# lingya/titan

Hardware: AMD Instinct MI355X
Metric: BFS GTEPS + PageRank s/iter, RMAT scale-24 (1 GPU) and scale-27 (1/2/4/8 GPU) (higher is better)
Workload: dtype int32 (BFS levels); f64 (PageRank)

## Files before the change

### titan_amd/csrc/api_msbfs.cpp

```cpp
#include <algorithm>
#include <cstdio>
#include <cstring>
#include "ctx.hpp"

using namespace tgo;

namespace tgo {

int ms_alloc(tgo_ctx* ctx) {
    Scratch& s = ctx->sc;
    if (s.ms_vis) return TGO_OK;
    const int64_t n = ctx->g.n;
    HIP_TRY(dev_alloc(ctx, s.ms_vis, n + 1));
    HIP_TRY(dev_alloc(ctx, s.ms_fr, n + 1));
    HIP_TRY(dev_alloc(ctx, s.ms_nx, n + 1));
    HIP_TRY(dev_alloc(ctx, s.ms_lvl, n * kLevelPlanes + 1));
    HIP_TRY(dev_alloc(ctx, s.ms_fbm, (n + 63) / 64 + 1));
    HIP_TRY(dev_alloc(ctx, s.ms_seeds, TGO_MAX_SOURCES));
    HIP_TRY(dev_alloc(ctx, s.ms_stat, 2 * TGO_MAX_SOURCES));
    HIP_TRY(dev_alloc(ctx, s.ms_srcent, TGO_MAX_SOURCES));
    ctx->st.device_bytes = ctx->dev_bytes;
    return TGO_OK;
}

double ms_split_of(const tgo_ctx* ctx) {
    static const double env = env_double("TGO_MS_SPLIT", 0.005);
    return tuned(ctx->tune.f64(TGO_TUNE_MS_SPLIT), env);
}
double ms_stay_of(const tgo_ctx* ctx) {
    static const double env = env_clamped("TGO_MS_STAY", kMsStayDefault, 0.0, HUGE_VAL);
    return tuned(ctx->tune.f64(TGO_TUNE_MS_STAY), env);
// ... 63 lines not shown
    s.ms_masks_zero = false;
    if (!masks_zero) HIP_TRY(hipMemsetAsync(s.ms_fr, 0, n * 8, st));
    s.ms_nplanes = 0;
    HIP_TRY(k_ms_seed(s.ms_seeds, nseeds, s.ms_vis, s.ms_fr, INT64_MAX, st));
    HIP_TRY(k_degree_i64(push, s.q[0], static_cast<int64_t>(uniq.size()), s.qdeg, st));
    const uint64_t full = nseeds == 64 ? ~0ULL : ((1ULL << nseeds) - 1ULL);
    const int64_t total = pull.nlists > 1 ? g.out.nnz + g.in.nnz : (scope == TGO_SCOPE_IN_E ? g.out.nnz : g.in.nnz);
    static const double ms_alpha = env_double("TGO_MS_ALPHA", 12.0);
    static const bool trace = trace_on();
    static const int32_t filter_from = env_double("TGO_MS_FILTER", 0.0) != 0.0
        ? 0 : static_cast<int32_t>(env_double("TGO_MS_FILTER_FROM", -1.0));
    const bool filter = filter_from >= 0 && filter_from < n;
    const double split_frac = tgo::ms_split_of(ctx);
    const double stay_gamma = tgo::ms_stay_of(ctx), sparse_frac = tgo::ms_sparse_of(ctx);
    const int64_t head = tgo::ms_head_of(ctx);
    int64_t qlen = static_cast<int64_t>(uniq.size());
    int64_t mf = 0;
    int64_t reached = qlen;
    bool srcent_ready = false;
    static const double push_light = env_double("TGO_MS_PUSH_LIGHT", 1.0 / 16.0);
    static const bool push_probe = env_double("TGO_MS_PUSH_PROBE", 1.0) != 0.0;
    static const int push_range_log2 = static_cast<int>(env_double("TGO_MS_PUSH_RANGE", 0.0));
    static const int64_t push_range_min = static_cast<int64_t>(env_double("TGO_MS_PUSH_RANGE_MIN", 1048576.0));
    const int depth = std::min(max_depth, 65534);
    uint64_t* fr = s.ms_fr;
    uint64_t* nx = s.ms_nx;
    int cur = 0, levels = 0;
    bool queued = true;
    bool pulled = false;
    bool cnt_zero = false;
    bool nx_clean = masks_zero;
    int64_t prev_mf = 0;
    int64_t mu = -1;
    bool level0_sparse = false, last_sparse = false;
    unsigned long long se_pub[TGO_MAX_SOURCES] = {};
    const volatile unsigned long long* hw = host_words(ctx);
    for (int L = 0; L < depth && qlen > 0; ++L) {
        const bool stay = pulled && mu >= 0 && stay_gamma > 0.0 &&
                          static_cast<double>(mu) <= stay_gamma * static_cast<double>(mf);
        const bool use_pull = stay || static_cast<double>(mf) * ms_alpha > static_cast<double>(total);
        DevSpan span(st, "msbfs.level", {"level", L}, {"pull", use_pull ? 1 : 0});
        if ((rc = ms_planes_for(ctx, L + 1))) return rc;
        const bool queued_before = queued;
        if (!use_pull && !queued) {
            if (!cnt_zero) HIP_TRY(hipMemsetAsync(s.cnt, 0, sizeof(Counters), st));
            HIP_TRY(k_ms_queue(push, g.n_active, fr, s.q[cur], s.qdeg, s.cnt, st));
        }
        queued = !use_pull;
        const bool prev_pull = pulled;
        pulled = use_pull;
        bool sums = false;
        if (!use_pull && !queued_before) cnt_zero = false;
        bool sparse_level = false;
        bool count_open = false;
        if (use_pull) {
            if (!cnt_zero) HIP_TRY(hipMemsetAsync(s.cnt, 0, sizeof(Counters), st));
            cnt_zero = true;
// ... 49 lines not shown
            }
            if (filter) HIP_TRY(k_ms_fbitmap(fr, n, s.ms_fbm, st));
            MsColdSplit cs;
            static const bool cold_env = env_double("TGO_MS_COLD", 0.0) != 0.0;
            const int64_t cold = ctx->tune.i64(TGO_TUNE_MS_COLD);
            const bool cold_on = tuned_on(cold, cold_env);
            if (cold_on && !prev_pull && !filter) {
                if ((rc = ms_cold_layout(ctx, scope, pull, cold))) return rc;
                if (g.msc_C > 0) {
                    cs.hot_lim = g.msc_hot;
                    cs.acc = s.ms_cacc;
                    cs.need = s.ms_need;
                }
            }
            count_open = stay_gamma > 0.0 && !cs.acc && mf < prev_mf;
            HIP_TRY(k_ms_pull(pull, push, g.n_active, full, fr, filter ? s.ms_fbm : nullptr, s.ms_vis, nx,
                              ms_planes(ctx), s.cnt, L + 1, st, filter ? filter_from : 0, full & ~sparse,
                              sparse ? nx : nullptr, cs, count_open, cs.acc ? 0 : head));
            if (cs.acc) {
                HIP_TRY(k_ms_cold(g.msc_adj, g.msc_row, g.msc_C, fr, s.ms_need, s.ms_cacc, st));
                HIP_TRY(k_ms_finish(push, g.n_active, full, s.ms_vis, nx, sparse ? nx : nullptr, ms_planes(ctx), s.cnt,
                                    L + 1, s.ms_need, s.ms_cacc, st));
            }
        } else {
            HIP_TRY(k_level_prep(cnt_zero ? nullptr : s.cnt, nx, nx_clean ? 0 : g.n_active, s.qdeg + qlen, st));
            cnt_zero = true;
            const int64_t rng = static_cast<int64_t>(1) << std::min(40, std::max(0, push_range_log2));
            const int64_t nr = (g.n_active + rng - 1) / rng;
            const bool ranged = push_range_log2 > 0 && mf >= push_range_min && nr > 1 &&
                                (nr + 1) * qlen <= kMsRangePairs && nr * qlen + 1 <= n + 2;
            sparse_level = sparse_frac > 0.0 && !ranged &&
                           (L == 0 || static_cast<double>(mf) <= sparse_frac * static_cast<double>(g.n_active));
            sums = split_frac > 0.0 && (L == 0 || static_cast<double>(mf) * ms_alpha * 64.0 > static_cast<double>(total));
// ... 22 lines not shown
            } else if (next_pull) {
                HIP_TRY(k_ms_settle_count(push, g.n_active, s.ms_vis, nx, ms_planes(ctx), s.cnt, L + 1, st,
                                          sums ? s.ms_srcent : nullptr));
                queued = false;
            } else {
                HIP_TRY(k_ms_settle(push, g.n_active, s.ms_vis, nx, ms_planes(ctx), s.q[cur ^ 1], s.qdeg, s.cnt, L + 1,
                                    st, sums ? s.ms_srcent : nullptr));
            }
        }
        srcent_ready = !use_pull && sums;
        {
            unsigned long long seq = 0;
            if ((rc = turn_begin(ctx, seq, sums ? s.ms_srcent : nullptr))) return rc;
            cnt_zero = true;
            if (sums) s.ms_srcent_zero = true;
            if (L + 1 < depth && (rc = ms_planes_for(ctx, L + 2))) return rc;
            if ((rc = wait_publish(ctx, seq))) return rc;
        }
        qlen = static_cast<int64_t>(s.hcnt->qlen);
        prev_mf = mf;
        mf = static_cast<int64_t>(s.hcnt->mf);
        mu = count_open ? static_cast<int64_t>(s.hcnt->open) : -1;
        if (sums)
            for (int r = 0; r < TGO_MAX_SOURCES; ++r) se_pub[r] = hw[kPublishExtra + r];
        reached += qlen;
        nx_clean = sparse_level;
        last_sparse = sparse_level;
        if (L == 0) level0_sparse = sparse_level;
        if (trace) std::fprintf(stderr, "[tgo] ms level %d %s -> %lld vertices, %lld entries, %llu source-bits%s\n", L,
                                use_pull ? "pull" : "push", (long long)qlen, (long long)mf, s.hcnt->red[0],
                                use_pull ? (stay ? " (stayed in pull)" : "") : (sparse_level ? " (sparse)" : ""));
        if (trace && count_open) std::fprintf(stderr, "[tgo]   %lld list entries of still-open vertices\n", (long long)mu);
        static const bool diag = env_double("TGO_MS_DIAG", 0.0) != 0.0;
        if (trace && diag && use_pull) {
            unsigned long long d[kMsDiagWords] = {};
            HIP_TRY(k_ms_diag_take(d, st));
            std::fprintf(stderr, "[tgo]   pull: %llu entries examined, %llu hot / %llu cold mask gathers, %llu open vertices, "
                         "%llu stopped early; long lists: %llu, %llu entries examined (%llu hot / %llu cold gathers), "
                         "%llu stopped early\n", d[0], d[1], d[2], d[3], d[4], d[6], d[5], d[8], d[9], d[7]);
            std::fprintf(stderr, "[tgo]   long lists covered within 4 / 8 / 16 / 32 / 64 entries: %llu / %llu / %llu / %llu / %llu, "
                         "later %llu, never %llu (head %lld)\n", d[10], d[11], d[12], d[13], d[14], d[15], d[16],
                         static_cast<long long>(head));
        }
        std::swap(fr, nx);
        cur ^= 1;
        ++levels;
    }
    if (qlen > 0 && max_depth > depth)
// ... 73 lines not shown
```

### titan_amd/csrc/ctx.hpp

```cpp
#pragma once
#include <algorithm>
#include <atomic>
#include <memory>
#include <string>
#include <utility>
#include <vector>
#include <hip/hip_runtime_api.h>
#include "engine.hpp"
#include "trace.hpp"
#include "tuning.hpp"
#include "../../include/titan_gpu_olap_part.h"

struct tgo_ctx {
    tgo_options opts{};
    hipStream_t stream = nullptr;
    bool own_stream = false;
    std::string err;
    tgo::RowStaging staging;
    tgo::DevGraph g;
    bool loaded = false;
    std::vector<int64_t> titan_id;
    std::vector<int32_t> perm;
    bool id_sorted = false;
    std::vector<std::pair<int64_t, int32_t>> id_index;
// ... 244 lines not shown
int run_bfs(tgo_ctx* ctx, int64_t seed, int max_depth, int scope);

int titan_ids_by_index(tgo_ctx* ctx);

int tri_forward_lists(tgo_ctx* ctx);

int ms_alloc(tgo_ctx* ctx);
double ms_split_of(const tgo_ctx* ctx);
double ms_stay_of(const tgo_ctx* ctx);
double ms_sparse_of(const tgo_ctx* ctx);
int64_t ms_head_of(const tgo_ctx* ctx);
int run_ms_sweep(tgo_ctx* ctx, const int64_t* seeds, int32_t nseeds, int32_t max_depth, int32_t scope, int32_t flags);

inline LevelPlanes ms_planes(tgo_ctx* ctx) { return LevelPlanes{ctx->sc.ms_lvl, ctx->g.n}; }

inline int ms_planes_for(tgo_ctx* ctx, int32_t level) {
    Scratch& s = ctx->sc;
    while (s.ms_nplanes < kLevelPlanes && (level >> s.ms_nplanes) != 0) {
        HIP_TRY(hipMemsetAsync(s.ms_lvl + static_cast<int64_t>(s.ms_nplanes) * ctx->g.n, 0,
                               ctx->g.n * sizeof(uint64_t), ctx->stream));
        ++s.ms_nplanes;
    }
    return TGO_OK;
}

}

#include "program.hpp"
```

### titan_amd/csrc/engine.hpp

```cpp
#pragma once
#include <algorithm>
#include <cstdint>
#include <string>
#include <vector>
#include <hip/hip_runtime_api.h>
#include "../../include/titan_gpu_olap.h"
#include "env.hpp"

namespace tgo {

template <class T>
struct DevArray {
    T* p = nullptr;
    int64_t n = -1;
    DevArray() = default;
    DevArray(const DevArray&) = delete;
    DevArray& operator=(const DevArray&) = delete;
    DevArray(DevArray&& o) noexcept : p(o.p), n(o.n) { o.p = nullptr; o.n = -1; }
    DevArray& operator=(DevArray&& o) noexcept {
        if (this != &o) { reset(); p = o.p; n = o.n; o.p = nullptr; o.n = -1; }
        return *this;
    }
    ~DevArray() { reset(); }
    void reset() { if (p) (void)hipFree(p); p = nullptr; n = -1; }
// ... 455 lines not shown
    void* cub_tmp = nullptr;
    size_t cub_bytes = 0;
    Counters* cnt = nullptr;
    Counters* hcnt = nullptr;
    unsigned long long* hcnt_dev = nullptr;
    unsigned long long pub_seq = 0;
    uint64_t* ms_vis = nullptr;
    uint64_t* ms_fbm = nullptr;
    unsigned long long* ms_srcent = nullptr;
    int64_t* ms_rp[2] = {nullptr, nullptr};
    uint64_t* ms_fr = nullptr;
    uint64_t* ms_nx = nullptr;
    uint64_t* ms_lvl = nullptr;
    int32_t ms_nplanes = 0;
    bool ms_masks_zero = false;
    bool ms_srcent_zero = false;
    int64_t* ms_seeds = nullptr;
    unsigned long long* ms_stat = nullptr;
    int32_t ms_nsrc = 0;
    unsigned long long* cl_far = nullptr;
    unsigned long long* cl_reach = nullptr;
    int32_t* cl_ecc = nullptr;
    double* cl_harm = nullptr;
    double* cl_close = nullptr;
    int* pk_ovf = nullptr;
    uint8_t* pk_touch = nullptr;
    int64_t* pk_cnt = nullptr;
    int64_t* pk_off = nullptr;
    int64_t* ds_light = nullptr;
    int64_t ds_light_delta = -1;
// ... 127 lines not shown
hipError_t k_ds_mark_pack(uint64_t* rmark, int64_t words, int64_t wpr, int64_t n_local, const int64_t* rbest,
                          const unsigned long long* offs, unsigned long long* cursor, int64_t* send, hipStream_t s);
hipError_t k_ds_mark_sizes(unsigned long long* counts, int nranks, int64_t qlen, unsigned long long* offs,
                           unsigned long long* cursor, const long long* track, int64_t* sizes, hipStream_t s);
hipError_t k_ds_apply(const View& push, const int64_t* recv, int64_t npairs, int64_t* dist, uint64_t* pend, int32_t* qn,
                      int64_t* qdeg_n, Counters* cnt, int64_t thr, const int64_t* ws_off, const int64_t* light,
                      long long* track, hipStream_t s);
hipError_t k_unpermute_i64(const int64_t* in, const int32_t* perm, int64_t* out, int64_t n, hipStream_t s);
hipError_t k_ms_seed(const int64_t* seeds, int nseeds, uint64_t* vis, uint64_t* fr, int64_t fr_rows, hipStream_t s);
constexpr int kMsDiagWords = 17;
hipError_t k_ms_diag_take(unsigned long long* out, hipStream_t s);
hipError_t k_ms_pull(const View& pull, const View& push, int64_t n_active, uint64_t full, const uint64_t* fr,
                     const uint64_t* fbm, uint64_t* vis, uint64_t* nx, LevelPlanes lvl, Counters* cnt,
                     int32_t next_level, hipStream_t s, int32_t filter_from, uint64_t dense = ~0ULL,
                     const uint64_t* cand = nullptr, MsColdSplit cs = MsColdSplit(), bool count_open = false,
                     int64_t head = 0);
hipError_t k_ms_cold(const int32_t* cadj, const int32_t* crow, int64_t C, const uint64_t* fr, const uint8_t* need,
                     uint64_t* acc, hipStream_t s);
hipError_t k_ms_finish(const View& push, int64_t n_active, uint64_t full, uint64_t* vis, uint64_t* nx,
                       const uint64_t* cand, LevelPlanes lvl, Counters* cnt, int32_t next_level, uint8_t* need,
                       const uint64_t* acc, hipStream_t s);
hipError_t k_cold_flags(const int32_t* adj, int64_t m, int32_t hot, uint32_t* flag, hipStream_t s);
hipError_t k_cold_emit(const int64_t* off, int64_t n, const int32_t* adj, int64_t m, const uint32_t* flag,
                       const uint64_t* pos, int64_t base, int32_t hot, int64_t seg, uint64_t* key, int32_t* val,
                       hipStream_t s);
hipError_t k_low_rows(const uint64_t* key, int64_t m, int32_t* row, hipStream_t s);
int build_ms_cold(const View& v, int64_t n, int32_t hot, int64_t seg, DevArray<int32_t>& cadj, DevArray<int32_t>& crow,
                  int64_t& C, hipStream_t s, std::string& err);
hipError_t k_ms_source_counts(const uint64_t* fr, int64_t n_active, unsigned long long* out64, hipStream_t s);
hipError_t k_ms_source_entries(const View& push, const uint64_t* fr, int64_t n_active, uint64_t cand,
                               unsigned long long* out64, hipStream_t s);
hipError_t k_ms_fbitmap(const uint64_t* fr, int64_t n, uint64_t* fbm, hipStream_t s);
hipError_t k_ms_queue(const View& push, int64_t n_active, const uint64_t* fr, int32_t* qn, int64_t* qdeg, Counters* cnt,
                      hipStream_t s, uint64_t mask = ~0ULL);
struct PackTouch { uint8_t* flag = nullptr; int64_t n_local = 1; int64_t cps = 1; };
hipError_t k_ms_push(const View& push, const int32_t* q, const int64_t* qpre, int64_t qlen, const uint64_t* fr,
                     const uint64_t* vis, uint64_t* nx, hipStream_t s, PackTouch touch = {}, uint64_t mask = ~0ULL,
                     bool probe = true, uint64_t* own_nx = nullptr, int64_t own_lo = 0);
constexpr double kMsStayDefault = 4.0;
constexpr double kMsSparseDefault = 1.0 / 16.0;
constexpr int64_t kMsHeadDefault = 4;
constexpr int64_t kMsHeadMax = 1 << 20;
hipError_t k_ms_push_sparse(const View& push, const int32_t* q, const int64_t* qpre, int64_t qlen, const uint64_t* fr,
                            const uint64_t* vis, uint64_t* nx, int32_t* qn, Counters* cnt, hipStream_t s);
hipError_t k_ms_settle_sparse(const View& push, const int32_t* qn, int64_t* qdeg, uint64_t* vis, const uint64_t* nx,
                              LevelPlanes lvl, Counters* cnt, int32_t next_level, hipStream_t s,
                              unsigned long long* srcent, const int32_t* qp, int64_t qplen, uint64_t* fr);
constexpr int64_t kMsRangePairs = int64_t(1) << 22;
hipError_t k_ms_push_ranged(const View& push, const int32_t* q, int64_t qlen, int64_t n_active, int64_t S,
                            int64_t* P0, int64_t* P1, int64_t* cnt, int64_t* pre, void*& tmp, size_t& tmp_bytes,
                            const uint64_t* fr, const uint64_t* vis, uint64_t* nx, hipStream_t s, uint64_t mask = ~0ULL);
hipError_t k_ms_settle_count(const View& push, int64_t n_active, uint64_t* vis, uint64_t* nx, LevelPlanes lvl,
                            Counters* cnt, int32_t next_level, hipStream_t s, unsigned long long* srcent = nullptr);
hipError_t k_ms_settle(const View& push, int64_t n_active, uint64_t* vis, uint64_t* nx, LevelPlanes lvl, int32_t* qn,
                       int64_t* qdeg, Counters* cnt, int32_t next_level, hipStream_t s,
                       unsigned long long* srcent = nullptr);
hipError_t k_ms_reach(const View& v, const uint64_t* vis, int64_t n_active, int nsrc, unsigned long long* reached,
// ... 201 lines not shown
```

### titan_amd/csrc/msbfs.hip

```cpp
#include <cstdlib>
#include <hip/hip_runtime.h>
#include "frontier.hpp"

namespace tgo {
namespace {

constexpr int kMaxSources = 64;

__device__ __forceinline__ int32_t view_entry(const View& v, int64_t u, int64_t o) {
    const int64_t b0 = v.off0[u];
    const int64_t d0 = v.off0[u + 1] - b0;
    return o < d0 ? v.adj0[b0 + o] : v.adj1[v.off1[u] + (o - d0)];
}

__device__ __forceinline__ void record_level(int64_t v, uint64_t fresh, int32_t level, const LevelPlanes& pl) {
    for (int k = 0; k < kLevelPlanes && (level >> k); ++k)
        if ((level >> k) & 1) pl.p[k * pl.stride + v] |= fresh;
}

__device__ __forceinline__ void count_flush(Counters* cnt, unsigned long long nv, unsigned long long mf,
                                            unsigned long long bits, unsigned long long mu = 0) {
    __shared__ unsigned long long s_nv[kWavesPerBlock], s_mf[kWavesPerBlock], s_bits[kWavesPerBlock], s_mu[kWavesPerBlock];
    for (int off = 32; off > 0; off >>= 1) {
        nv += __shfl_xor(nv, off, 64);
// ... 74 lines not shown
            uint64_t m = 0;
#pragma unroll
            for (int j = 0; j < kStep; ++j) m |= f[j] ? mk[j] : 0ULL;
            acc |= m;
            if (kDiag)
                for (int j = 0; j < kStep; ++j)
                    if (ok[j]) { ++dg[dg_ent]; ++dg[u[j] < kDiagHot ? dg_hot : dg_hot + 1]; }
        }
        const int64_t reached = min(k, e);
        lim -= reached - from;
        if (l == 0) k0 = reached; else k1 = reached;
        cut |= cutl;
    }
}

template <int kStep, bool kDiag = false, int kLong = 4, bool kRamp = false>
__global__ void __launch_bounds__(kBlock) ms_pull(View pull, View push, int64_t n_active, uint64_t full,
        const uint64_t* __restrict__ fr, const uint64_t* __restrict__ fbm, uint64_t* __restrict__ vis,
        uint64_t* __restrict__ nx, LevelPlanes lvl, Counters* cnt, int32_t next_level, int32_t filter_from,
        uint64_t dense, const uint64_t* __restrict__ cand, MsColdSplit cs, int64_t coop, bool count_open, int64_t head) {
    const int32_t hot_lim = cs.hot_lim;
    unsigned long long nv = 0, mf = 0, bits = 0, mu = 0;
    unsigned long long dg[kDiagWords] = {};
    const int64_t words = (n_active + 63) >> 6;
    for (int64_t b = static_cast<int64_t>(blockIdx.x) * kWavesPerBlock; b < words; b += static_cast<int64_t>(gridDim.x) * kWavesPerBlock) {
        const int64_t wd = b + (threadIdx.x >> 6);
        const int64_t v = (wd << 6) + lane();
        const uint64_t seen = v < n_active ? vis[v] : full;
        const uint64_t open = full & ~seen;
        const uint64_t want = open & dense;
        int64_t b0 = 0, e0 = 0, b1 = 0, e1 = 0;
        if (open) {
            b0 = pull.off0[v]; e0 = pull.off0[v + 1];
            if (pull.nlists > 1) { b1 = pull.off1[v]; e1 = pull.off1[v + 1]; }
        }
        const int64_t deg = (e0 - b0) + (e1 - b1);
        const bool is_big = want != 0 && deg > coop;
        uint64_t acc = 0;
        bool cut = false;
        int64_t h0 = b0, h1 = b1;
        if (want)
            walk_own<kStep, kDiag>(pull, h0, e0, h1, e1, is_big ? head : INT64_MAX, want, fr, fbm, filter_from, hot_lim,
                                   acc, cut, dg, is_big ? 5 : 0, is_big ? 8 : 1);
        const bool head_done = is_big && (acc & want) == want;
        if (kDiag) {
            if (want && !is_big) { ++dg[3]; if ((acc & want) == want) ++dg[4]; }
            if (head_done) { ++dg[6]; ++dg[7]; ++dg[diag_cover_bucket((h0 - b0) + (h1 - b1))]; }
        }
        unsigned long long big = __ballot(is_big && !head_done);
        while (big) {
            const int src = __ffsll(static_cast<long long>(big)) - 1;
            big &= big - 1;
            const uint64_t wsrc = __shfl(want, src, 64);
            uint64_t a = __shfl(acc, src, 64);
            bool wcut = false;
            int64_t pos = kDiag ? __shfl((h0 - b0) + (h1 - b1), src, 64) : 0;
            int64_t cover = -1;
            for (int l = 0; l < 2; ++l) {
                const int64_t bb = __shfl(l == 0 ? h0 : h1, src, 64);
                const int64_t ee = __shfl(l == 0 ? e0 : e1, src, 64);
                const int32_t* adj = l == 0 ? pull.adj0 : pull.adj1;
                bool done = false;
                bool first = kRamp && l == 0;
                for (int64_t k = bb; k < ee && !done;) {
                    const int jl = first ? 1 : kLong;
                    int32_t u[kLong];
                    bool hc = false;
#pragma unroll
                    for (int j = 0; j < kLong; ++j) {
                        const int64_t x = k + j * 64 + lane();
                        u[j] = (j < jl && x < ee) ? __builtin_nontemporal_load(adj + x) : -1;
                        if (u[j] >= hot_lim) { u[j] = -1; hc = true; }
                    }
                    const int64_t trip = min(static_cast<int64_t>(jl) * 64, ee - k);
                    k += static_cast<int64_t>(jl) * 64;
                    first = false;
                    if (__ballot(hc)) { done = true; wcut = true; }
                    bool f[kLong];
#pragma unroll
                    for (int j = 0; j < kLong; ++j) f[j] = u[j] >= 0 && maybe_frontier(fbm, u[j], filter_from);
                    uint64_t m = 0;
#pragma unroll
                    for (int j = 0; j < kLong; ++j)
                        if (f[j]) m |= fr[u[j]];
                    if (kDiag && cover < 0) {
                        uint64_t p = m;
                        for (int o = 1; o < 64; o <<= 1) {
                            const uint64_t y = __shfl_up(p, o, 64);
                            if (lane() >= o) p |= y;
                        }
                        const unsigned long long cv = __ballot(((a | p) & wsrc) == wsrc);
                        if (cv) cover = pos + (kLong == 1 ? __ffsll(static_cast<long long>(cv)) : trip);
                        pos += trip;
                    }
                    for (int off = 32; off > 0; off >>= 1) m |= __shfl_xor(m, off, 64);
                    if (kDiag)
                        for (int j = 0; j < kLong; ++j)
                            if (u[j] >= 0) ++dg[u[j] < kDiagHot ? 8 : 9];
                    a |= m;
                    done = done || (a & wsrc) == wsrc;
                    if (kDiag && lane() == src)
                        for (int j = 0; j < kLong; ++j) dg[5] += u[j] >= 0 ? 1 : 0;
                }
                if ((a & wsrc) == wsrc) break;
            }
            if (lane() == src) {
                acc = a;
                cut = wcut;
                if (kDiag) {
                    ++dg[6];
                    if ((a & wsrc) == wsrc) ++dg[7];
                    ++dg[(a & wsrc) == wsrc && cover >= 0 ? diag_cover_bucket(cover) : 16];
                }
            }
        }
        if (cut && (acc & want) != want && v < n_active) {
            cs.acc[v] = acc;
            cs.need[v] = 1;
            continue;
        }
        if (cand && open && v < n_active) acc |= cand[v];
        const uint64_t fresh = acc & open;
        if (v < n_active) {
            nx[v] = fresh;
            if (fresh) vis[v] = seen | fresh;
        }
        if (fresh) {
            record_level(v, fresh, next_level, lvl);
            ++nv;
            mf += static_cast<unsigned long long>(push_degree(push, v));
            bits += static_cast<unsigned long long>(__popcll(fresh));
        }
        if (count_open && (open & ~fresh)) mu += static_cast<unsigned long long>(deg);
    }
    if (kDiag) {
        for (int i = 0; i < kDiagWords; ++i) {
            unsigned long long x = dg[i];
            for (int off = 32; off > 0; off >>= 1) x += __shfl_xor(x, off, 64);
            if (lane() == 0 && x) atomicAdd(&g_ms_diag[i], x);
        }
    }
    count_flush(cnt, nv, mf, bits, mu);
}

__global__ void __launch_bounds__(kBlock) ms_cold(const int32_t* __restrict__ cadj, const int32_t* __restrict__ crow,
        int64_t C, const uint64_t* __restrict__ fr, const uint8_t* __restrict__ need, uint64_t* __restrict__ acc) {
    const int x = static_cast<int>(blockIdx.x & 7u);
    const int64_t per = gridDim.x >> 3;
    const int64_t lo = C * x / 8, hi = C * (x + 1) / 8;
    const int64_t span = (hi - lo + 63) & ~int64_t(63);
    for (int64_t e0 = lo + static_cast<int64_t>(blockIdx.x >> 3) * kBlock; e0 < lo + span; e0 += per * kBlock) {
        const int64_t e = e0 + threadIdx.x;
        int32_t v = -1;
        uint64_t m = 0;
        if (e < hi) {
// ... 651 lines not shown
    int64_t g = (work + kBlock - 1) / kBlock;
    if (g < 1) g = 1;
    if (g > cap) g = cap;
    return static_cast<int>(g);
}

}

hipError_t k_ms_seed(const int64_t* seeds, int nseeds, uint64_t* vis, uint64_t* fr, int64_t fr_rows, hipStream_t s) {
    ms_seed<<<1, 64, 0, s>>>(seeds, nseeds, vis, fr, fr_rows);
    return hipGetLastError();
}
hipError_t k_ms_pull(const View& pull, const View& push, int64_t n_active, uint64_t full, const uint64_t* fr,
                     const uint64_t* fbm, uint64_t* vis, uint64_t* nx, LevelPlanes lvl, Counters* cnt,
                     int32_t next_level, hipStream_t s, int32_t filter_from, uint64_t dense, const uint64_t* cand,
                     MsColdSplit cs, bool count_open, int64_t head) {
    static const int step = static_cast<int>(env_i64("TGO_MS_STEP", 4));
    static const bool diag = env_i64("TGO_MS_DIAG", 0) != 0;
    static const int lng = static_cast<int>(env_i64("TGO_MS_LONG", 1));
    static const bool ramp = env_i64("TGO_MS_RAMP", 0) != 0;
    static const int64_t coop = env_i64("TGO_MS_COOP", kCoop);
    const dim3 grid(grid_for(n_active, 8192));
#define TGO_MS_PULL(S, D, LG, R) ms_pull<S, D, LG, R><<<grid, kBlock, 0, s>>>(pull, push, n_active, full, fr, fbm, vis, \
        nx, lvl, cnt, next_level, filter_from, dense, cand, cs, coop, count_open, head)
    if (diag) TGO_MS_PULL(4, true, 1, false);
    else if (ramp) TGO_MS_PULL(8, false, 4, true);
    else if (step == 4 && lng == 1) TGO_MS_PULL(4, false, 1, false);
    else if (step == 16 && lng == 1) TGO_MS_PULL(16, false, 1, false);
    else if (lng == 1) TGO_MS_PULL(8, false, 1, false);
    else if (lng == 2) TGO_MS_PULL(8, false, 2, false);
    else if (lng == 8) TGO_MS_PULL(8, false, 8, false);
    else if (step == 4) TGO_MS_PULL(4, false, 4, false);
    else if (step == 16) TGO_MS_PULL(16, false, 4, false);
    else TGO_MS_PULL(8, false, 4, false);
#undef TGO_MS_PULL
    return hipGetLastError();
// ... 159 lines not shown
```

### titan_amd/csrc/trace.cpp

```cpp
#include "trace.hpp"

#include <chrono>
#include <cstdio>
#include <cstdlib>
#include <cstring>
#include <mutex>
#include <thread>
#include <vector>

#include <rocprofiler-sdk-roctx/roctx.h>

#include "../../include/titan_gpu_olap.h"

namespace tgo {

std::atomic<int> g_trace_flags{0};

namespace {

struct Event {
    std::string name;
    double ts = 0, dur = 0;
    uint64_t tid = 0;
    int dev = 0;
    TraceArg a{nullptr, 0}, b{nullptr, 0};
};
struct Pending {
    hipStream_t s;
    std::string name;
    TraceArg a, b;
    hipEvent_t e0, e1;
};

struct State {
    std::mutex mu;
    std::vector<Event> events;
    std::vector<Pending> pending;
    std::vector<hipEvent_t> pool;
    std::string path;
    std::chrono::steady_clock::time_point base = std::chrono::steady_clock::now();
    bool atexit_set = false;
};
State& st() {
    static State* s = new State();
    return *s;
// ... 23 lines not shown

int write_json(const char* path) {
    State& S = st();
    std::lock_guard<std::mutex> lk(S.mu);
    std::FILE* f = std::fopen(path, "w");
    if (!f) return TGO_E_INVALID;
    std::fprintf(f, "{\"displayTimeUnit\": \"ms\", \"otherData\": {\"producer\": \"titan_amd\"}, \"traceEvents\": [\n");
    for (size_t i = 0; i < S.events.size(); ++i) {
        const Event& e = S.events[i];
        std::fprintf(f, "{\"name\": \"");
        json_escape(f, e.name);
        std::fprintf(f, "\", \"cat\": \"%s\", \"ph\": \"X\", \"ts\": %.3f, \"dur\": %.3f, \"pid\": %d, \"tid\": %llu",
                     e.dev ? "device" : "host", e.ts, e.dur, e.dev ? 1 : 0, static_cast<unsigned long long>(e.tid));
        std::fprintf(f, ", \"args\": {");
        bool first = true;
        for (const TraceArg& a : {e.a, e.b}) {
            if (!a.key) continue;
            std::fprintf(f, "%s\"%s\": %lld", first ? "" : ", ", a.key, static_cast<long long>(a.value));
            first = false;
        }
        std::fprintf(f, "}}%s\n", i + 1 < S.events.size() ? "," : "");
    }
    std::fprintf(f, "]}\n");
    return std::fclose(f) == 0 ? TGO_OK : TGO_E_INVALID;
}

void flush_at_exit() {
    State& S = st();
    if (!S.path.empty() && (g_trace_flags.load() & kTraceJson)) (void)write_json(S.path.c_str());
}

// ... 20 lines not shown
Span::~Span() {
    if (roctx_) roctxRangePop();
    if (t0_ < 0) return;
    Event e;
    e.name = name_;
    e.ts = static_cast<double>(t0_) / 1000.0;
    e.dur = now_us() - e.ts;
    e.tid = tid_now();
    e.a = a_;
    e.b = b_;
    State& S = st();
    std::lock_guard<std::mutex> lk(S.mu);
    S.events.push_back(std::move(e));
}

DevSpan::DevSpan(hipStream_t s, const char* name, TraceArg a, TraceArg b) : s_(s), name_(name), a_(a), b_(b) {
    const int f = g_trace_flags.load(std::memory_order_relaxed);
    if (!f) return;
    if (f & kTraceRoctx) { roctxRangePushA(name); roctx_ = true; }
    if (f & kTraceJson) {
        e0_ = take_event();
        e1_ = take_event();
        if (e0_ && e1_ && hipEventRecord(e0_, s_) == hipSuccess) open_ = true;
    }
}
void DevSpan::end() {
    if (roctx_) { roctxRangePop(); roctx_ = false; }
    if (!open_) return;
    open_ = false;
    if (hipEventRecord(e1_, s_) != hipSuccess) return;
    State& S = st();
    std::lock_guard<std::mutex> lk(S.mu);
    S.pending.push_back({s_, name_, a_, b_, e0_, e1_});
}

void trace_complete(const std::string& name, double dur_us) {
    if (!(g_trace_flags.load(std::memory_order_relaxed) & kTraceJson)) return;
    Event e;
    e.name = name;
    e.dur = dur_us;
    e.ts = now_us() - dur_us;
    e.tid = tid_now();
    State& S = st();
    std::lock_guard<std::mutex> lk(S.mu);
    S.events.push_back(std::move(e));
}

void trace_resolve(hipStream_t s) {
// ... 12 lines not shown
    if (!ref || hipEventRecord(ref, s) != hipSuccess || hipEventSynchronize(ref) != hipSuccess) return;
    const double host_ref = now_us();
    const uint64_t tid = 0x1000000ULL + (reinterpret_cast<uintptr_t>(s) & 0xFFFFFF);
    std::vector<Event> out;
    for (const Pending& p : mine) {
        float a = 0.f, d = 0.f;
        if (hipEventElapsedTime(&a, p.e0, ref) != hipSuccess || hipEventElapsedTime(&d, p.e0, p.e1) != hipSuccess) continue;
        Event e;
        e.name = p.name;
        e.ts = host_ref - static_cast<double>(a) * 1000.0;
        e.dur = static_cast<double>(d) * 1000.0;
        e.tid = tid;
        e.dev = 1;
        e.a = p.a;
        e.b = p.b;
        out.push_back(std::move(e));
    }
    std::lock_guard<std::mutex> lk(S.mu);
    for (auto& e : out) S.events.push_back(std::move(e));
    for (const Pending& p : mine) { S.pool.push_back(p.e0); S.pool.push_back(p.e1); }
    S.pool.push_back(ref);
}

}

using namespace tgo;

extern "C" {

int tgo_trace_enable(const char* json_path, int32_t flags) {
// ... 57 lines not shown
```

### titan_amd/csrc/trace.hpp

```cpp
#pragma once
#include <atomic>
#include <cstdint>
#include <string>

#include <hip/hip_runtime.h>

namespace tgo {

enum : int { kTraceJson = 1, kTraceRoctx = 2 };
extern std::atomic<int> g_trace_flags;
inline bool tracing() { return g_trace_flags.load(std::memory_order_relaxed) != 0; }

struct TraceArg {
    const char* key;
    int64_t value;
};

class Span {
public:
    Span(const char* name, TraceArg a = {nullptr, 0}, TraceArg b = {nullptr, 0});
    ~Span();
    Span(const Span&) = delete;
    Span& operator=(const Span&) = delete;
private:
    const char* name_;
    TraceArg a_, b_;
    int64_t t0_ = -1;
    bool roctx_ = false;
};

class DevSpan {
public:
    DevSpan(hipStream_t s, const char* name, TraceArg a = {nullptr, 0}, TraceArg b = {nullptr, 0});
    ~DevSpan() { end(); }
    void end();
    DevSpan(const DevSpan&) = delete;
    DevSpan& operator=(const DevSpan&) = delete;
private:
    hipStream_t s_;
    const char* name_;
    TraceArg a_, b_;
    hipEvent_t e0_ = nullptr, e1_ = nullptr;
    bool roctx_ = false, open_ = false;
};

void trace_complete(const std::string& name, double dur_us);

void trace_resolve(hipStream_t s);

}
```

Before: 5512.

## Compact open vertices in late MS-BFS pull levels and skip redundant plane clears

Measured after the change: 5841 (median of 6 runs). +6.0%, better.

```diff
diff --git a/titan_amd/csrc/api_msbfs.cpp b/titan_amd/csrc/api_msbfs.cpp
--- a/titan_amd/csrc/api_msbfs.cpp
+++ b/titan_amd/csrc/api_msbfs.cpp
@@ -15,6 +15,11 @@
     HIP_TRY(dev_alloc(ctx, s.ms_fr, n + 1));
     HIP_TRY(dev_alloc(ctx, s.ms_nx, n + 1));
     HIP_TRY(dev_alloc(ctx, s.ms_lvl, n * kLevelPlanes + 1));
+    s.ms_clean = 0;
+    if (n > ctx->g.n_active)
+        for (int k = 0; k < kLevelPlanes; ++k)
+            HIP_TRY(hipMemsetAsync(s.ms_lvl + static_cast<int64_t>(k) * n + ctx->g.n_active, 0,
+                                   (n - ctx->g.n_active) * sizeof(uint64_t), ctx->stream));
     HIP_TRY(dev_alloc(ctx, s.ms_fbm, (n + 63) / 64 + 1));
     HIP_TRY(dev_alloc(ctx, s.ms_seeds, TGO_MAX_SOURCES));
     HIP_TRY(dev_alloc(ctx, s.ms_stat, 2 * TGO_MAX_SOURCES));
@@ -108,6 +113,12 @@
     const double split_frac = tgo::ms_split_of(ctx);
     const double stay_gamma = tgo::ms_stay_of(ctx), sparse_frac = tgo::ms_sparse_of(ctx);
     const int64_t head = tgo::ms_head_of(ctx);
+    static const bool diag = env_double("TGO_MS_DIAG", 0.0) != 0.0;
+    static const bool compact_on = env_i64("TGO_MS_COMPACT", 1) != 0 && !diag;
+    static const int32_t compact_chunk = [] {
+        const int64_t c = env_i64("TGO_MS_CHUNK", kMsChunkDefault);
+        return static_cast<int32_t>(c == 512 || c == 1024 || c == 2048 ? c : kMsChunkDefault);
+    }();
     int64_t qlen = static_cast<int64_t>(uniq.size());
     int64_t mf = 0;
     int64_t reached = qlen;
@@ -133,8 +144,10 @@
         const bool stay = pulled && mu >= 0 && stay_gamma > 0.0 &&
                           static_cast<double>(mu) <= stay_gamma * static_cast<double>(mf);
         const bool use_pull = stay || static_cast<double>(mf) * ms_alpha > static_cast<double>(total);
-        DevSpan span(st, "msbfs.level", {"level", L}, {"pull", use_pull ? 1 : 0});
-        if ((rc = ms_planes_for(ctx, L + 1))) return rc;
+        DevSpan span(st, "msbfs.level", {"level", L}, {"pull", use_pull ? 1 : 0}, {"compact", 0});
+        if ((rc = ms_planes_for(ctx, L + 1, true))) return rc;
+        const uint32_t was_clean = s.ms_clean & ms_planes_written(L + 1);
+        s.ms_clean &= ~was_clean;
         const bool queued_before = queued;
         if (!use_pull && !queued) {
             if (!cnt_zero) HIP_TRY(hipMemsetAsync(s.cnt, 0, sizeof(Counters), st));
@@ -214,9 +227,12 @@
                 }
             }
             count_open = stay_gamma > 0.0 && !cs.acc && mf < prev_mf;
+            const bool compact = compact_on && count_open && !sparse;
+            if (compact) span.set_third(1);
             HIP_TRY(k_ms_pull(pull, push, g.n_active, full, fr, filter ? s.ms_fbm : nullptr, s.ms_vis, nx,
                               ms_planes(ctx), s.cnt, L + 1, st, filter ? filter_from : 0, full & ~sparse,
-                              sparse ? nx : nullptr, cs, count_open, cs.acc ? 0 : head));
+                              sparse ? nx : nullptr, cs, count_open, cs.acc ? 0 : head,
+                              compact ? compact_chunk : 0));
             if (cs.acc) {
                 HIP_TRY(k_ms_cold(g.msc_adj, g.msc_row, g.msc_C, fr, s.ms_need, s.ms_cacc, st));
                 HIP_TRY(k_ms_finish(push, g.n_active, full, s.ms_vis, nx, sparse ? nx : nullptr, ms_planes(ctx), s.cnt,
@@ -269,10 +285,11 @@
             if ((rc = turn_begin(ctx, seq, sums ? s.ms_srcent : nullptr))) return rc;
             cnt_zero = true;
             if (sums) s.ms_srcent_zero = true;
-            if (L + 1 < depth && (rc = ms_planes_for(ctx, L + 2))) return rc;
+            if (L + 1 < depth && (rc = ms_planes_for(ctx, L + 2, true))) return rc;
             if ((rc = wait_publish(ctx, seq))) return rc;
         }
         qlen = static_cast<int64_t>(s.hcnt->qlen);
+        if (qlen == 0) s.ms_clean |= was_clean;
         prev_mf = mf;
         mf = static_cast<int64_t>(s.hcnt->mf);
         mu = count_open ? static_cast<int64_t>(s.hcnt->open) : -1;
@@ -286,7 +303,6 @@
                                 use_pull ? "pull" : "push", (long long)qlen, (long long)mf, s.hcnt->red[0],
                                 use_pull ? (stay ? " (stayed in pull)" : "") : (sparse_level ? " (sparse)" : ""));
         if (trace && count_open) std::fprintf(stderr, "[tgo]   %lld list entries of still-open vertices\n", (long long)mu);
-        static const bool diag = env_double("TGO_MS_DIAG", 0.0) != 0.0;
         if (trace && diag && use_pull) {
             unsigned long long d[kMsDiagWords] = {};
             HIP_TRY(k_ms_diag_take(d, st));
diff --git a/titan_amd/csrc/ctx.hpp b/titan_amd/csrc/ctx.hpp
--- a/titan_amd/csrc/ctx.hpp
+++ b/titan_amd/csrc/ctx.hpp
@@ -282,15 +282,24 @@
 
 inline LevelPlanes ms_planes(tgo_ctx* ctx) { return LevelPlanes{ctx->sc.ms_lvl, ctx->g.n}; }
 
-inline int ms_planes_for(tgo_ctx* ctx, int32_t level) {
+inline int ms_planes_for(tgo_ctx* ctx, int32_t level, bool keep_clean = false) {
     Scratch& s = ctx->sc;
     while (s.ms_nplanes < kLevelPlanes && (level >> s.ms_nplanes) != 0) {
-        HIP_TRY(hipMemsetAsync(s.ms_lvl + static_cast<int64_t>(s.ms_nplanes) * ctx->g.n, 0,
-                               ctx->g.n * sizeof(uint64_t), ctx->stream));
+        const uint32_t bit = 1u << s.ms_nplanes;
+        uint64_t* plane = s.ms_lvl + static_cast<int64_t>(s.ms_nplanes) * ctx->g.n;
+        if (!keep_clean) {
+            s.ms_clean &= ~bit;
+            HIP_TRY(hipMemsetAsync(plane, 0, ctx->g.n * sizeof(uint64_t), ctx->stream));
+        } else if (!(s.ms_clean & bit)) {
+            const int64_t rows = std::min<int64_t>(ctx->g.n, (ctx->g.n_active + 511) & ~int64_t(511));
+            if (rows > 0) HIP_TRY(hipMemsetAsync(plane, 0, rows * sizeof(uint64_t), ctx->stream));
+            s.ms_clean |= bit;
+        }
         ++s.ms_nplanes;
     }
     return TGO_OK;
 }
+inline uint32_t ms_planes_written(int32_t level) { return static_cast<uint32_t>(level) & ((1u << kLevelPlanes) - 1u); }
 
 }
 
diff --git a/titan_amd/csrc/engine.hpp b/titan_amd/csrc/engine.hpp
--- a/titan_amd/csrc/engine.hpp
+++ b/titan_amd/csrc/engine.hpp
@@ -493,6 +493,7 @@
     uint64_t* ms_lvl = nullptr;
     int32_t ms_nplanes = 0;
     bool ms_masks_zero = false;
+    uint32_t ms_clean = 0;
     bool ms_srcent_zero = false;
     int64_t* ms_seeds = nullptr;
     unsigned long long* ms_stat = nullptr;
@@ -650,7 +651,7 @@
                      const uint64_t* fbm, uint64_t* vis, uint64_t* nx, LevelPlanes lvl, Counters* cnt,
                      int32_t next_level, hipStream_t s, int32_t filter_from, uint64_t dense = ~0ULL,
                      const uint64_t* cand = nullptr, MsColdSplit cs = MsColdSplit(), bool count_open = false,
-                     int64_t head = 0);
+                     int64_t head = 0, int32_t compact_chunk = 0);
 hipError_t k_ms_cold(const int32_t* cadj, const int32_t* crow, int64_t C, const uint64_t* fr, const uint8_t* need,
                      uint64_t* acc, hipStream_t s);
 hipError_t k_ms_finish(const View& push, int64_t n_active, uint64_t full, uint64_t* vis, uint64_t* nx,
@@ -677,6 +678,7 @@
 constexpr double kMsSparseDefault = 1.0 / 16.0;
 constexpr int64_t kMsHeadDefault = 4;
 constexpr int64_t kMsHeadMax = 1 << 20;
+constexpr int64_t kMsChunkDefault = 1024;
 hipError_t k_ms_push_sparse(const View& push, const int32_t* q, const int64_t* qpre, int64_t qlen, const uint64_t* fr,
                             const uint64_t* vis, uint64_t* nx, int32_t* qn, Counters* cnt, hipStream_t s);
 hipError_t k_ms_settle_sparse(const View& push, const int32_t* qn, int64_t* qdeg, uint64_t* vis, const uint64_t* nx,
diff --git a/titan_amd/csrc/msbfs.hip b/titan_amd/csrc/msbfs.hip
--- a/titan_amd/csrc/msbfs.hip
+++ b/titan_amd/csrc/msbfs.hip
@@ -1,3 +1,4 @@
+#include <algorithm>
 #include <cstdlib>
 #include <hip/hip_runtime.h>
 #include "frontier.hpp"
@@ -112,12 +113,126 @@
     }
 }
 
+template <int kStep, bool kDiag, int kLong, bool kRamp>
+__device__ __forceinline__ void pull_vertex(const View& pull, const View& push, int64_t n_active, uint64_t full,
+        const uint64_t* __restrict__ fr, const uint64_t* __restrict__ fbm, uint64_t* __restrict__ vis,
+        uint64_t* __restrict__ nx, const LevelPlanes& lvl, int32_t next_level, int32_t filter_from, uint64_t dense,
+        const uint64_t* __restrict__ cand, const MsColdSplit& cs, int64_t coop, bool count_open, int64_t head,
+        int64_t v, uint64_t seen, unsigned long long& nv, unsigned long long& mf, unsigned long long& bits,
+        unsigned long long& mu, unsigned long long* dg) {
+    const int32_t hot_lim = cs.hot_lim;
+    const uint64_t open = full & ~seen;
+    const uint64_t want = open & dense;
+    int64_t b0 = 0, e0 = 0, b1 = 0, e1 = 0;
+    if (open) {
+        b0 = pull.off0[v]; e0 = pull.off0[v + 1];
+        if (pull.nlists > 1) { b1 = pull.off1[v]; e1 = pull.off1[v + 1]; }
+    }
+    const int64_t deg = (e0 - b0) + (e1 - b1);
+    const bool is_big = want != 0 && deg > coop;
+    uint64_t acc = 0;
+    bool cut = false;
+    int64_t h0 = b0, h1 = b1;
+    if (want)
+        walk_own<kStep, kDiag>(pull, h0, e0, h1, e1, is_big ? head : INT64_MAX, want, fr, fbm, filter_from, hot_lim,
+                               acc, cut, dg, is_big ? 5 : 0, is_big ? 8 : 1);
+    const bool head_done = is_big && (acc & want) == want;
+    if (kDiag) {
+        if (want && !is_big) { ++dg[3]; if ((acc & want) == want) ++dg[4]; }
+        if (head_done) { ++dg[6]; ++dg[7]; ++dg[diag_cover_bucket((h0 - b0) + (h1 - b1))]; }
+    }
+    unsigned long long big = __ballot(is_big && !head_done);
+    while (big) {
+        const int src = __ffsll(static_cast<long long>(big)) - 1;
+        big &= big - 1;
+        const uint64_t wsrc = __shfl(want, src, 64);
+        uint64_t a = __shfl(acc, src, 64);
+        bool wcut = false;
+        int64_t pos = kDiag ? __shfl((h0 - b0) + (h1 - b1), src, 64) : 0;
+        int64_t cover = -1;
+        for (int l = 0; l < 2; ++l) {
+            const int64_t bb = __shfl(l == 0 ? h0 : h1, src, 64);
+            const int64_t ee = __shfl(l == 0 ? e0 : e1, src, 64);
+            const int32_t* adj = l == 0 ? pull.adj0 : pull.adj1;
+            bool done = false;
+            bool first = kRamp && l == 0;
+            for (int64_t k = bb; k < ee && !done;) {
+                const int jl = first ? 1 : kLong;
+                int32_t u[kLong];
+                bool hc = false;
+#pragma unroll
+                for (int j = 0; j < kLong; ++j) {
+                    const int64_t x = k + j * 64 + lane();
+                    u[j] = (j < jl && x < ee) ? __builtin_nontemporal_load(adj + x) : -1;
+                    if (u[j] >= hot_lim) { u[j] = -1; hc = true; }
+                }
+                const int64_t trip = min(static_cast<int64_t>(jl) * 64, ee - k);
+                k += static_cast<int64_t>(jl) * 64;
+                first = false;
+                if (__ballot(hc)) { done = true; wcut = true; }
+                bool f[kLong];
+#pragma unroll
+                for (int j = 0; j < kLong; ++j) f[j] = u[j] >= 0 && maybe_frontier(fbm, u[j], filter_from);
+                uint64_t m = 0;
+#pragma unroll
+                for (int j = 0; j < kLong; ++j)
+                    if (f[j]) m |= fr[u[j]];
+                if (kDiag && cover < 0) {
+                    uint64_t p = m;
+                    for (int o = 1; o < 64; o <<= 1) {
+                        const uint64_t y = __shfl_up(p, o, 64);
+                        if (lane() >= o) p |= y;
+                    }
+                    const unsigned long long cv = __ballot(((a | p) & wsrc) == wsrc);
+                    if (cv) cover = pos + (kLong == 1 ? __ffsll(static_cast<long long>(cv)) : trip);
+                    pos += trip;
+                }
+                for (int off = 32; off > 0; off >>= 1) m |= __shfl_xor(m, off, 64);
+                if (kDiag)
+                    for (int j = 0; j < kLong; ++j)
+                        if (u[j] >= 0) ++dg[u[j] < kDiagHot ? 8 : 9];
+                a |= m;
+                done = done || (a & wsrc) == wsrc;
+                if (kDiag && lane() == src)
+                    for (int j = 0; j < kLong; ++j) dg[5] += u[j] >= 0 ? 1 : 0;
+            }
+            if ((a & wsrc) == wsrc) break;
+        }
+        if (lane() == src) {
+            acc = a;
+            cut = wcut;
+            if (kDiag) {
+                ++dg[6];
+                if ((a & wsrc) == wsrc) ++dg[7];
+                ++dg[(a & wsrc) == wsrc && cover >= 0 ? diag_cover_bucket(cover) : 16];
+            }
+        }
+    }
+    if (cut && (acc & want) != want && v < n_active) {
+        cs.acc[v] = acc;
+        cs.need[v] = 1;
+        return;
+    }
+    if (cand && open && v < n_active) acc |= cand[v];
+    const uint64_t fresh = acc & open;
+    if (v < n_active) {
+        nx[v] = fresh;
+        if (fresh) vis[v] = seen | fresh;
+    }
+    if (fresh) {
+        record_level(v, fresh, next_level, lvl);
+        ++nv;
+        mf += static_cast<unsigned long long>(push_degree(push, v));
+        bits += static_cast<unsigned long long>(__popcll(fresh));
+    }
+    if (count_open && (open & ~fresh)) mu += static_cast<unsigned long long>(deg);
+}
+
 template <int kStep, bool kDiag = false, int kLong = 4, bool kRamp = false>
 __global__ void __launch_bounds__(kBlock) ms_pull(View pull, View push, int64_t n_active, uint64_t full,
         const uint64_t* __restrict__ fr, const uint64_t* __restrict__ fbm, uint64_t* __restrict__ vis,
         uint64_t* __restrict__ nx, LevelPlanes lvl, Counters* cnt, int32_t next_level, int32_t filter_from,
         uint64_t dense, const uint64_t* __restrict__ cand, MsColdSplit cs, int64_t coop, bool count_open, int64_t head) {
-    const int32_t hot_lim = cs.hot_lim;
     unsigned long long nv = 0, mf = 0, bits = 0, mu = 0;
     unsigned long long dg[kDiagWords] = {};
     const int64_t words = (n_active + 63) >> 6;
@@ -125,111 +240,8 @@
         const int64_t wd = b + (threadIdx.x >> 6);
         const int64_t v = (wd << 6) + lane();
         const uint64_t seen = v < n_active ? vis[v] : full;
-        const uint64_t open = full & ~seen;
-        const uint64_t want = open & dense;
-        int64_t b0 = 0, e0 = 0, b1 = 0, e1 = 0;
-        if (open) {
-            b0 = pull.off0[v]; e0 = pull.off0[v + 1];
-            if (pull.nlists > 1) { b1 = pull.off1[v]; e1 = pull.off1[v + 1]; }
-        }
-        const int64_t deg = (e0 - b0) + (e1 - b1);
-        const bool is_big = want != 0 && deg > coop;
-        uint64_t acc = 0;
-        bool cut = false;
-        int64_t h0 = b0, h1 = b1;
-        if (want)
-            walk_own<kStep, kDiag>(pull, h0, e0, h1, e1, is_big ? head : INT64_MAX, want, fr, fbm, filter_from, hot_lim,
-                                   acc, cut, dg, is_big ? 5 : 0, is_big ? 8 : 1);
-        const bool head_done = is_big && (acc & want) == want;
-        if (kDiag) {
-            if (want && !is_big) { ++dg[3]; if ((acc & want) == want) ++dg[4]; }
-            if (head_done) { ++dg[6]; ++dg[7]; ++dg[diag_cover_bucket((h0 - b0) + (h1 - b1))]; }
-        }
-        unsigned long long big = __ballot(is_big && !head_done);
-        while (big) {
-            const int src = __ffsll(static_cast<long long>(big)) - 1;
-            big &= big - 1;
-            const uint64_t wsrc = __shfl(want, src, 64);
-            uint64_t a = __shfl(acc, src, 64);
-            bool wcut = false;
-            int64_t pos = kDiag ? __shfl((h0 - b0) + (h1 - b1), src, 64) : 0;
-            int64_t cover = -1;
-            for (int l = 0; l < 2; ++l) {
-                const int64_t bb = __shfl(l == 0 ? h0 : h1, src, 64);
-                const int64_t ee = __shfl(l == 0 ? e0 : e1, src, 64);
-                const int32_t* adj = l == 0 ? pull.adj0 : pull.adj1;
-                bool done = false;
-                bool first = kRamp && l == 0;
-                for (int64_t k = bb; k < ee && !done;) {
-                    const int jl = first ? 1 : kLong;
-                    int32_t u[kLong];
-                    bool hc = false;
-#pragma unroll
-                    for (int j = 0; j < kLong; ++j) {
-                        const int64_t x = k + j * 64 + lane();
-                        u[j] = (j < jl && x < ee) ? __builtin_nontemporal_load(adj + x) : -1;
-                        if (u[j] >= hot_lim) { u[j] = -1; hc = true; }
-                    }
-                    const int64_t trip = min(static_cast<int64_t>(jl) * 64, ee - k);
-                    k += static_cast<int64_t>(jl) * 64;
-                    first = false;
-                    if (__ballot(hc)) { done = true; wcut = true; }
-                    bool f[kLong];
-#pragma unroll
-                    for (int j = 0; j < kLong; ++j) f[j] = u[j] >= 0 && maybe_frontier(fbm, u[j], filter_from);
-                    uint64_t m = 0;
-#pragma unroll
-                    for (int j = 0; j < kLong; ++j)
-                        if (f[j]) m |= fr[u[j]];
-                    if (kDiag && cover < 0) {
-                        uint64_t p = m;
-                        for (int o = 1; o < 64; o <<= 1) {
-                            const uint64_t y = __shfl_up(p, o, 64);
-                            if (lane() >= o) p |= y;
-                        }
-                        const unsigned long long cv = __ballot(((a | p) & wsrc) == wsrc);
-                        if (cv) cover = pos + (kLong == 1 ? __ffsll(static_cast<long long>(cv)) : trip);
-                        pos += trip;
-                    }
-                    for (int off = 32; off > 0; off >>= 1) m |= __shfl_xor(m, off, 64);
-                    if (kDiag)
-                        for (int j = 0; j < kLong; ++j)
-                            if (u[j] >= 0) ++dg[u[j] < kDiagHot ? 8 : 9];
-                    a |= m;
-                    done = done || (a & wsrc) == wsrc;
-                    if (kDiag && lane() == src)
-                        for (int j = 0; j < kLong; ++j) dg[5] += u[j] >= 0 ? 1 : 0;
-                }
-                if ((a & wsrc) == wsrc) break;
-            }
-            if (lane() == src) {
-                acc = a;
-                cut = wcut;
-                if (kDiag) {
-                    ++dg[6];
-                    if ((a & wsrc) == wsrc) ++dg[7];
-                    ++dg[(a & wsrc) == wsrc && cover >= 0 ? diag_cover_bucket(cover) : 16];
-                }
-            }
-        }
-        if (cut && (acc & want) != want && v < n_active) {
-            cs.acc[v] = acc;
-            cs.need[v] = 1;
-            continue;
-        }
-        if (cand && open && v < n_active) acc |= cand[v];
-        const uint64_t fresh = acc & open;
-        if (v < n_active) {
-            nx[v] = fresh;
-            if (fresh) vis[v] = seen | fresh;
-        }
-        if (fresh) {
-            record_level(v, fresh, next_level, lvl);
-            ++nv;
-            mf += static_cast<unsigned long long>(push_degree(push, v));
-            bits += static_cast<unsigned long long>(__popcll(fresh));
-        }
-        if (count_open && (open & ~fresh)) mu += static_cast<unsigned long long>(deg);
+        pull_vertex<kStep, kDiag, kLong, kRamp>(pull, push, n_active, full, fr, fbm, vis, nx, lvl, next_level, filter_from,
+                                                dense, cand, cs, coop, count_open, head, v, seen, nv, mf, bits, mu, dg);
     }
     if (kDiag) {
         for (int i = 0; i < kDiagWords; ++i) {
@@ -237,6 +249,62 @@
             for (int off = 32; off > 0; off >>= 1) x += __shfl_xor(x, off, 64);
             if (lane() == 0 && x) atomicAdd(&g_ms_diag[i], x);
         }
+    }
+    count_flush(cnt, nv, mf, bits, mu);
+}
+
+constexpr int kCompactScan = 8;
+template <int kStep, int kLong>
+__global__ void __launch_bounds__(kBlock) ms_pull_compact(View pull, View push, int64_t n_active, uint64_t full,
+        const uint64_t* __restrict__ fr, const uint64_t* __restrict__ fbm, uint64_t* __restrict__ vis,
+        uint64_t* __restrict__ nx, LevelPlanes lvl, Counters* cnt, int32_t next_level, int32_t filter_from,
+        int64_t coop, bool count_open, int64_t head, int32_t chunk) {
+    extern __shared__ int32_t s_open[];
+    unsigned long long nv = 0, mf = 0, bits = 0, mu = 0;
+    const MsColdSplit cs;
+    const int64_t words = (n_active + 63) >> 6;
+    const int32_t per = chunk >> 6;
+    const int64_t chunks = (words + per - 1) / per;
+    const int64_t last = n_active > 0 ? n_active - 1 : 0;
+    const unsigned long long below = (1ULL << lane()) - 1ULL;
+    const int wave = __builtin_amdgcn_readfirstlane(static_cast<int>(threadIdx.x >> 6));
+    int32_t* ids = s_open + wave * chunk;
+    for (int64_t c = static_cast<int64_t>(blockIdx.x) * kWavesPerBlock + wave; c < chunks;
+         c += static_cast<int64_t>(gridDim.x) * kWavesPerBlock) {
+        int32_t nopen = 0;
+        for (int32_t w = 0; w < per; w += kCompactScan) {
+            uint64_t sv[kCompactScan];
+#pragma unroll
+            for (int j = 0; j < kCompactScan; ++j) {
+                const int64_t wd = min(c + (w + j) * chunks, words - 1);
+                const int32_t lim = static_cast<int32_t>(min(last - (wd << 6), static_cast<int64_t>(63)));
+                sv[j] = (vis + (wd << 6))[min(lane(), lim)];
+            }
+#pragma unroll
+            for (int j = 0; j < kCompactScan; ++j) {
+                const int64_t wd = c + (w + j) * chunks;
+                const int64_t v = (wd << 6) + lane();
+                const bool live = wd < words && v < n_active;
+                const bool is_open = live && (full & ~sv[j]) != 0;
+                if (live && !is_open) nx[v] = 0;
+                const unsigned long long m = __ballot(is_open);
+                if (is_open) ids[nopen + __popcll(m & below)] = static_cast<int32_t>(v);
+                nopen += __popcll(m);
+            }
+        }
+        __builtin_amdgcn_fence(__ATOMIC_RELEASE, "wavefront");
+        __builtin_amdgcn_wave_barrier();
+        __builtin_amdgcn_fence(__ATOMIC_ACQUIRE, "wavefront");
+        for (int32_t i = 0; i < nopen; i += 64) {
+            const bool has = i + lane() < nopen;
+            const int64_t v = has ? ids[i + lane()] : n_active;
+            const uint64_t got = vis[min(v, last)];
+            const uint64_t seen = has ? got : full;
+            pull_vertex<kStep, false, kLong, false>(pull, push, n_active, full, fr, fbm, vis, nx, lvl, next_level,
+                                                    filter_from, full, nullptr, cs, coop, count_open, head, v, seen, nv, mf,
+                                                    bits, mu, nullptr);
+        }
+        __builtin_amdgcn_wave_barrier();
     }
     count_flush(cnt, nv, mf, bits, mu);
 }
@@ -918,12 +986,22 @@
 hipError_t k_ms_pull(const View& pull, const View& push, int64_t n_active, uint64_t full, const uint64_t* fr,
                      const uint64_t* fbm, uint64_t* vis, uint64_t* nx, LevelPlanes lvl, Counters* cnt,
                      int32_t next_level, hipStream_t s, int32_t filter_from, uint64_t dense, const uint64_t* cand,
-                     MsColdSplit cs, bool count_open, int64_t head) {
+                     MsColdSplit cs, bool count_open, int64_t head, int32_t compact_chunk) {
+    static const int64_t coop_env = env_i64("TGO_MS_COOP", kCoop);
+    if (compact_chunk > 0) {
+        if (dense != full || cand || cs.acc || compact_chunk % (64 * kCompactScan) != 0) return hipErrorInvalidValue;
+        const int64_t chunks = ((n_active + 63) / 64 + compact_chunk / 64 - 1) / (compact_chunk / 64);
+        const int64_t blocks = std::min<int64_t>(std::max<int64_t>((chunks + kWavesPerBlock - 1) / kWavesPerBlock, 1), 8192);
+        const size_t lds = static_cast<size_t>(kWavesPerBlock) * compact_chunk * sizeof(int32_t);
+        ms_pull_compact<4, 1><<<static_cast<int>(blocks), kBlock, lds, s>>>(pull, push, n_active, full, fr, fbm, vis, nx,
+                lvl, cnt, next_level, filter_from, coop_env, count_open, head, compact_chunk);
+        return hipGetLastError();
+    }
     static const int step = static_cast<int>(env_i64("TGO_MS_STEP", 4));
     static const bool diag = env_i64("TGO_MS_DIAG", 0) != 0;
     static const int lng = static_cast<int>(env_i64("TGO_MS_LONG", 1));
     static const bool ramp = env_i64("TGO_MS_RAMP", 0) != 0;
-    static const int64_t coop = env_i64("TGO_MS_COOP", kCoop);
+    const int64_t coop = coop_env;
     const dim3 grid(grid_for(n_active, 8192));
 #define TGO_MS_PULL(S, D, LG, R) ms_pull<S, D, LG, R><<<grid, kBlock, 0, s>>>(pull, push, n_active, full, fr, fbm, vis, \
         nx, lvl, cnt, next_level, filter_from, dense, cand, cs, coop, count_open, head)
diff --git a/titan_amd/csrc/trace.cpp b/titan_amd/csrc/trace.cpp
--- a/titan_amd/csrc/trace.cpp
+++ b/titan_amd/csrc/trace.cpp
@@ -23,12 +23,12 @@
     double ts = 0, dur = 0;
     uint64_t tid = 0;
     int dev = 0;
-    TraceArg a{nullptr, 0}, b{nullptr, 0};
+    TraceArg a{nullptr, 0}, b{nullptr, 0}, c{nullptr, 0};
 };
 struct Pending {
     hipStream_t s;
     std::string name;
-    TraceArg a, b;
+    TraceArg a, b, c;
     hipEvent_t e0, e1;
 };
 
@@ -82,7 +82,7 @@
                      e.dev ? "device" : "host", e.ts, e.dur, e.dev ? 1 : 0, static_cast<unsigned long long>(e.tid));
         std::fprintf(f, ", \"args\": {");
         bool first = true;
-        for (const TraceArg& a : {e.a, e.b}) {
+        for (const TraceArg& a : {e.a, e.b, e.c}) {
             if (!a.key) continue;
             std::fprintf(f, "%s\"%s\": %lld", first ? "" : ", ", a.key, static_cast<long long>(a.value));
             first = false;
@@ -133,7 +133,8 @@
     S.events.push_back(std::move(e));
 }
 
-DevSpan::DevSpan(hipStream_t s, const char* name, TraceArg a, TraceArg b) : s_(s), name_(name), a_(a), b_(b) {
+DevSpan::DevSpan(hipStream_t s, const char* name, TraceArg a, TraceArg b, TraceArg c)
+    : s_(s), name_(name), a_(a), b_(b), c_(c) {
     const int f = g_trace_flags.load(std::memory_order_relaxed);
     if (!f) return;
     if (f & kTraceRoctx) { roctxRangePushA(name); roctx_ = true; }
@@ -150,7 +151,7 @@
     if (hipEventRecord(e1_, s_) != hipSuccess) return;
     State& S = st();
     std::lock_guard<std::mutex> lk(S.mu);
-    S.pending.push_back({s_, name_, a_, b_, e0_, e1_});
+    S.pending.push_back({s_, name_, a_, b_, c_, e0_, e1_});
 }
 
 void trace_complete(const std::string& name, double dur_us) {
@@ -193,6 +194,7 @@
         e.dev = 1;
         e.a = p.a;
         e.b = p.b;
+        e.c = p.c;
         out.push_back(std::move(e));
     }
     std::lock_guard<std::mutex> lk(S.mu);
diff --git a/titan_amd/csrc/trace.hpp b/titan_amd/csrc/trace.hpp
--- a/titan_amd/csrc/trace.hpp
+++ b/titan_amd/csrc/trace.hpp
@@ -31,15 +31,17 @@
 
 class DevSpan {
 public:
-    DevSpan(hipStream_t s, const char* name, TraceArg a = {nullptr, 0}, TraceArg b = {nullptr, 0});
+    DevSpan(hipStream_t s, const char* name, TraceArg a = {nullptr, 0}, TraceArg b = {nullptr, 0},
+            TraceArg c = {nullptr, 0});
     ~DevSpan() { end(); }
     void end();
+    void set_third(int64_t value) { c_.value = value; }
     DevSpan(const DevSpan&) = delete;
     DevSpan& operator=(const DevSpan&) = delete;
 private:
     hipStream_t s_;
     const char* name_;
-    TraceArg a_, b_;
+    TraceArg a_, b_, c_;
     hipEvent_t e0_ = nullptr, e1_ = nullptr;
     bool roctx_ = false, open_ = false;
 };
```
